# Trippasch/CudaRayTracer

Hardware: AMD Instinct MI355X
Metric: Mray/s (and ms/frame) at 1920x1080, 64 spp, depth 8, random-spheres (higher is better)
Workload: dtype f32; 1 GPU; c2: 1920x1080, 64 spp, depth 8, RTIOW final random-spheres scene; width=1920, height=1080, spp=64, depth=8, parallelism=1 GPU, kernel_variant=-1

## Files before the change

cudaraytracer_amd/_lib.py:

```python
from __future__ import annotations

import ctypes as C
import os

from . import abi

LIB_PATH = _IN_TREE = os.path.join(os.path.dirname(os.path.abspath(__file__)), "librt_hip.so")
LIB_PATH = os.environ.get("RT_HIP_LIB", LIB_PATH)

EXPORTED = [
    "LaunchKernel",
    "LaunchRandInit",
    "LaunchRenderInit",
    "rt_last_error",
    "rt_version",
    "rt_abi_version",
    "rt_set_launch_flags",
    "rt_set_device",
    "rt_scene_create",
    "rt_scene_from_reference_graph",
    "rt_scene_update_materials",
    "rt_scene_destroy",
    "rt_scene_get_info",
    "rt_render_init",
    "rt_render_init_soa",
    "rt_soa_plane_words",
    "rt_render",
    "rt_tiled_create",
    "rt_tiled_render",
    "rt_tiled_destroy",
    "rt_gl_register_texture",
    "rt_gl_copy_image",
    "rt_gl_unregister",
    "rt_copy_image_to_host",
    "rt_write_ppm",
    "rt_set_timing",
    "rt_set_wave_trace",
    "rt_set_tile_order",
    "rt_set_pixel_cost",
    "rt_set_ray_dump",
    "rt_trace_rays",
    "rt_query_rays",
    "rt_gbuffer",
    "rt_denoise",
    "rt_denoise_scratch_bytes",
    "rt_temporal",
    "rt_temporal_dynamic",
    "rt_temporal_moments",
    "rt_denoise_variance",
    "rt_denoise_variance_scratch_bytes",
    "rt_scene_motion",
    "rt_scene_edit",
    "rt_last_kernel_ms",
    "rt_last_variant",
    "rt_last_launch_host_ms",
    "rt_set_variant",
    "rt_set_tuning",
    "rt_glibc_srand",
    "rt_glibc_rand_next",
    "rt_builtin_scene",
    "rt_camera_inputs",
    "rt_procedural_texture",
    "rt_reference_graph_flatten",
    "rt_build_host_tables",
    "rt_tile_entries_host",
    "rt_set_bounce_entries",
    "rt_bounce_entries_host",
    "rt_bounce_entry_cells",
]

_lib = None


class RTError(RuntimeError):
    pass


def _declare(lib: C.CDLL) -> None:
    P = C.POINTER
    vp = C.c_void_p
    lib.rt_last_error.restype = C.c_char_p
    lib.rt_version.restype = C.c_char_p
    lib.rt_set_launch_flags.argtypes = [C.c_uint32]
    lib.rt_set_device.argtypes = [C.c_int]
    lib.rt_scene_create.argtypes = [P(abi.SceneDesc), P(vp)]
    lib.rt_scene_from_reference_graph.argtypes = [vp, P(vp)]
    lib.rt_scene_update_materials.argtypes = [vp, P(abi.MaterialDesc), C.c_uint32]
    lib.rt_scene_destroy.argtypes = [vp]
    lib.rt_scene_get_info.argtypes = [vp, P(abi.SceneInfo)]
    lib.rt_render_init.argtypes = [vp, C.c_uint32, C.c_uint32, P(abi.Tiling), C.c_uint64, vp]
    lib.rt_render_init_soa.argtypes = [vp, C.c_uint32, C.c_uint32, P(abi.Tiling), C.c_uint64, vp]
    lib.rt_soa_plane_words.argtypes = [C.c_uint32, C.c_uint32]
    lib.rt_soa_plane_words.restype = C.c_uint64
    lib.rt_render.argtypes = [vp, P(abi.RenderArgs), vp]
    lib.rt_set_timing.argtypes = [C.c_int]
    lib.rt_tiled_create.argtypes = [P(abi.TiledDesc), P(abi.SceneDesc), P(vp)]
    lib.rt_tiled_render.argtypes = [vp, P(abi.TiledFrame), P(abi.TiledTiming)]
    lib.rt_tiled_destroy.argtypes = [vp]
    lib.rt_gl_register_texture.argtypes = [C.c_uint32, C.c_uint32, P(vp)]
    lib.rt_gl_copy_image.argtypes = [vp, vp, C.c_uint32, C.c_uint32, vp]
    lib.rt_gl_unregister.argtypes = [vp]
    lib.rt_copy_image_to_host.argtypes = [vp, vp, C.c_uint32, C.c_uint32, C.c_int, vp]
    lib.rt_write_ppm.argtypes = [C.c_char_p, vp, C.c_uint32, C.c_uint32, C.c_int]
    lib.rt_set_wave_trace.argtypes = [C.c_void_p, C.c_uint64]
    lib.rt_set_tile_order.argtypes = [C.c_void_p]
    lib.rt_set_pixel_cost.argtypes = [C.c_void_p, C.c_uint64]
    lib.rt_set_ray_dump.argtypes = [C.c_void_p, C.c_uint32, C.c_void_p, C.c_uint32]
    lib.rt_trace_rays.argtypes = [C.c_void_p, C.c_void_p, C.c_uint32, C.c_void_p, C.c_void_p, C.c_int, C.c_void_p]
    if LIB_PATH == _IN_TREE or hasattr(lib, "rt_query_rays"):
        lib.rt_query_rays.argtypes = [vp, P(abi.QueryArgs), vp]
    lib.rt_gbuffer.argtypes = [vp, P(abi.GBufferArgs), vp]
    lib.rt_denoise.argtypes = [P(abi.DenoiseArgs), vp]
    lib.rt_denoise_scratch_bytes.argtypes = [C.c_uint32, C.c_uint32, C.c_uint32]
    lib.rt_denoise_scratch_bytes.restype = C.c_uint64
    lib.rt_temporal.argtypes = [P(abi.TemporalArgs), vp]
    lib.rt_temporal_dynamic.argtypes = [P(abi.TemporalArgs), vp, C.c_uint32, vp]
    lib.rt_temporal_moments.argtypes = [P(abi.TemporalArgs), vp, C.c_uint32, vp, vp, vp]
    lib.rt_denoise_variance.argtypes = [P(abi.DenoiseVarianceArgs), vp]
    lib.rt_denoise_variance_scratch_bytes.argtypes = [C.c_uint32, C.c_uint32, C.c_uint32]
    lib.rt_denoise_variance_scratch_bytes.restype = C.c_uint64
    lib.rt_scene_motion.argtypes = [P(abi.HittableDesc), P(abi.HittableDesc), C.c_uint32, P(C.c_float)]
    lib.rt_scene_edit.argtypes = [vp, P(abi.HittableDesc), C.c_uint32, P(vp)]
    lib.rt_last_kernel_ms.restype = C.c_float
    lib.rt_last_variant.restype = C.c_int
    lib.rt_last_launch_host_ms.restype = C.c_float
    lib.rt_set_variant.argtypes = [C.c_int]
    lib.rt_set_tuning.argtypes = [C.c_int, C.c_int]
    lib.rt_glibc_srand.argtypes = [P(abi.GlibcRand), C.c_uint32]
    lib.rt_glibc_rand_next.argtypes = [P(abi.GlibcRand)]
    lib.rt_glibc_rand_next.restype = C.c_int32
    lib.rt_builtin_scene.argtypes = [C.c_int, C.c_uint32, P(abi.HittableDesc), P(C.c_uint32),
                                     P(abi.MaterialDesc), P(C.c_uint32)]
    lib.rt_procedural_texture.argtypes = [C.c_int, C.c_int32, C.c_int32, C.c_void_p]
    F3P = P(C.c_float)
    lib.rt_camera_inputs.argtypes = [F3P, F3P, F3P, C.c_float, C.c_float, C.c_float, F3P, F3P, P(abi.InputStruct)]
    lib.rt_reference_graph_flatten.argtypes = [vp, P(abi.HittableDesc), P(C.c_uint32), P(abi.MaterialDesc),
                                               P(C.c_uint32), P(abi.ImageDesc), P(C.c_uint32)]
    lib.rt_build_host_tables.argtypes = [P(abi.SceneDesc), P(C.c_float), P(C.c_float), P(C.c_float),
                                         P(C.c_int32), P(abi.HostTablesInfo)]
    if LIB_PATH == _IN_TREE or hasattr(lib, "rt_tile_entries_host"):
        lib.rt_tile_entries_host.argtypes = [P(abi.SceneDesc), P(abi.InputStruct), C.c_uint32, C.c_uint32, P(abi.Tiling),
                                             C.c_uint32, C.c_uint32, C.c_uint32, P(C.c_uint32)]
    if LIB_PATH == _IN_TREE or hasattr(lib, "rt_set_bounce_entries"):
        lib.rt_set_bounce_entries.argtypes = [C.c_int]
        lib.rt_bounce_entries_host.argtypes = [P(abi.SceneDesc), P(C.c_float), P(C.c_float), P(C.c_uint32), P(C.c_uint32),
                                               P(C.c_uint16), P(abi.BounceEntriesInfo)]
        lib.rt_bounce_entry_cells.argtypes = [P(abi.BounceEntriesInfo), P(C.c_float), C.c_uint32, P(C.c_uint32)]
    lib.LaunchKernel.argtypes = [vp, C.c_uint, C.c_uint, C.c_uint, C.c_uint, vp, vp, abi.InputStruct]
    lib.LaunchKernel.restype = None
    lib.LaunchRandInit.argtypes = [vp]
    lib.LaunchRandInit.restype = None
    lib.LaunchRenderInit.argtypes = [abi.Dim3, abi.Dim3, C.c_uint, C.c_uint, vp]
    lib.LaunchRenderInit.restype = None


def lib() -> C.CDLL:
    global _lib
    if _lib is None:
        if not os.path.exists(LIB_PATH):
            raise RTError(f"{LIB_PATH} is missing: build it with `python -c 'import __graft_entry__ as g; g.build()'`")
        handle = C.CDLL(LIB_PATH)
        _declare(handle)
        _lib = handle
    return _lib


def check(rc: int, what: str) -> None:
    if rc != 0:
        msg = lib().rt_last_error().decode(errors="replace")
        raise RTError(f"{what} failed: {abi.STATUS.get(rc, rc)}: {msg}")
```

cudaraytracer_amd/csrc/render.hip:

```cpp
#include <hip/hip_runtime.h>

#include <cfloat>
#include <cstdio>
#include <cstdlib>
#include <cstring>
#include <atomic>
#include <map>
#include <numeric>
#include <memory>
#include <mutex>
#include <tuple>
#include <type_traits>
#include <vector>

#include "rt_epilogue.h"
#include "rt_internal.h"
#include "rt_scene_device.h"
#include "rt_tile_entry.h"

namespace rt {
namespace dev {

struct f3 {
    float x, y, z;
// ... 3381 lines not shown
    __syncthreads();
    for (uint32_t i = threadIdx.x; i < n; i += 1024u) order[atomicAdd(&start[cost_bucket(cost[i])], 1u)] = i;
}

__global__ __launch_bounds__(64) void tile_entries_kernel(const float* __restrict__ nodes, const float* __restrict__ prims,
                                                          const TileFrame F, TileRecord* __restrict__ out, const uint32_t n) {
    const uint32_t tile = blockIdx.x * 64u + threadIdx.x;
    if (tile < n) out[tile] = tile_record(nodes, prims, F, tile);
}

__global__ void rand_init_kernel(uint32_t* state) {
    if (threadIdx.x == 0 && blockIdx.x == 0) curand_init_state(1984ull, state);
}

}

namespace {

thread_local bool g_timing = false;
thread_local float g_last_ms = -1.0f;
thread_local float g_last_host_ms = -1.0f;
thread_local int g_variant = -1;
thread_local int g_last_variant = -1;

thread_local int g_regen_threshold = 56;
thread_local int g_regen_live_frac = 48;
thread_local int g_leaf_break = 3;
thread_local int g_lds_pad = 0;
thread_local int g_adaptive_order = 1;
thread_local int g_flat_max = 16;
thread_local int g_rius_trips = 4;
thread_local int g_rius_trips_persistent = 0;
thread_local int g_prefetch_stop = (int)dev::kPrefetchStop;
thread_local int g_persistent_waves = 0;
constexpr uint32_t kQueueMaxStride = 4096;
thread_local int g_queue_stride = 128;
thread_local int g_queue_chunk = 128;
thread_local int g_queue_prefetch = 32;
thread_local int g_queue_guide = 0;
thread_local int g_queue_min = 16;
thread_local int g_queue_host_reset = 0;
thread_local int g_persistent_group = 2;
thread_local int g_group_tail = 0;
thread_local int g_group_order = 0;
thread_local int g_group_chunk = 1024;
thread_local int g_group_waves = 16;
thread_local int g_group_linger_us = 0;
thread_local int g_tile_entries = 1;
thread_local int g_camera_resolve = 1;
constexpr uint32_t kCameraResolveCap = 8;
constexpr int kCameraResolveMax = 32;
thread_local int g_path_end_step = 1;
thread_local int g_bounce_entries = 1;

struct Knob {
    int& (*at)();
    int lo, hi, step;
    bool pow2;
    const char* refusal;
};
const Knob kKnobs[] = {
    {[]() -> int& { return g_regen_threshold; }, 1, 64, 1, false, "rt_set_tuning: regen threshold must be in [1, 64]"},
    {[]() -> int& { return g_leaf_max; }, 1, kLeafMax, 1, false, "rt_set_tuning: leaf max must be in [1, 4]"},
    {[]() -> int& { return g_persistent_waves; }, 0, 16, 1, false,
     "rt_set_tuning: persistent waves per SIMD must be in [0, 16]"},
    {[]() -> int& { return g_sah_traversal_x10; }, 1, 1000, 1, false,
     "rt_set_tuning: SAH traversal cost (x10) must be in [1, 1000]"},
    {[]() -> int& { return g_lds_pad; }, 0, 65536, 4, false, "rt_set_tuning: LDS pad must be a multiple of 4 in [0, 65536]"},
    {[]() -> int& { return g_adaptive_order; }, 0, 1, 1, false, "rt_set_tuning: adaptive order must be 0 or 1"},
    {[]() -> int& { return g_texel_bytes; }, 3, 4, 1, false, "rt_set_tuning: texel layout must be 3 (RGB8) or 4 (RGBA8)"},
    {[]() -> int& { return g_queue_chunk; }, 64, 4096, 64, false,
     "rt_set_tuning: queue chunk must be a multiple of 64 in [64, 4096]"},
    {[]() -> int& { return g_queue_stride; }, 128, (int)kQueueMaxStride, 1, true,
     "rt_set_tuning: queue head stride must be a power of two in [128, 4096] bytes"},
    {[]() -> int& { return g_regen_live_frac; }, 0, 64, 1, false, "rt_set_tuning: live fraction must be in [0, 64]"},
    {[]() -> int& { return g_leaf_break; }, 0, 64, 1, false, "rt_set_tuning: leaf break must be in [0, 64]"},
    {[]() -> int& { return g_rius_trips; }, 0, 64, 1, false, "rt_set_tuning: RandomInUnitSphere trips must be in [0, 64]"},
    {[]() -> int& { return g_flat_max; }, 0, (int)kFlatMaxPrims, 1, false,
     "rt_set_tuning: flat kernel primitive limit must be in [0, 64]"},
    {[]() -> int& { return g_queue_prefetch; }, 0, 64, 1, false, "rt_set_tuning: queue prefetch must be in [0, 64]"},
    {[]() -> int& { return g_queue_guide; }, 0, 64, 1, false, "rt_set_tuning: queue guide factor must be in [0, 64]"},
    {[]() -> int& { return g_queue_min; }, 16, 64, 16, false, "rt_set_tuning: guided chunk floor must be 16, 32, 48 or 64"},
    {[]() -> int& { return g_rius_trips_persistent; }, 0, 64, 1, false,
     "rt_set_tuning: RandomInUnitSphere trips must be in [0, 64]"},
    {[]() -> int& { return g_prefetch_stop; }, 0, 1024, 1, false, "rt_set_tuning: prefetch stop must be in [0, 1024]"},
    {[]() -> int& { return g_persistent_group; }, 0, 2, 1, false, "rt_set_tuning: persistent group must be 0, 1 or 2"},
    {[]() -> int& { return g_group_tail; }, 0, 1000, 1, false, "rt_set_tuning: group tail must be in [0, 1000] permille"},
    {[]() -> int& { return g_group_order; }, 0, 1, 1, false, "rt_set_tuning: group order must be 0 or 1"},
    {[]() -> int& { return g_queue_host_reset; }, 0, 1, 1, false, "rt_set_tuning: queue reset must be 0 or 1"},
    {[]() -> int& { return g_group_chunk; }, 64, 4096, 64, false,
     "rt_set_tuning: group chunk must be a multiple of 64 in [64, 4096]"},
    {[]() -> int& { return g_group_linger_us; }, 0, 100000, 1, false,
     "rt_set_tuning: group linger must be in [0, 100000] us"},
    {[]() -> int& { return g_group_waves; }, 4, 16, 4, false, "rt_set_tuning: group waves must be 4, 8, 12 or 16"},
    {[]() -> int& { return g_tile_entries; }, 0, 1, 1, false, "rt_set_tuning: tile entries must be 0 or 1"},
    {[]() -> int& { return g_camera_resolve; }, 0, kCameraResolveMax, 1, false,
     "rt_set_tuning: camera resolve must be 0, 1 or a primitive cap in [2, 32]"},
    {[]() -> int& { return g_path_end_step; }, 0, 1, 1, false, "rt_set_tuning: path end step must be 0 or 1"},
};
static_assert(sizeof(kKnobs) / sizeof(kKnobs[0]) == RT_TUNE_PATH_END_STEP + 1, "one row per rt_tuning_key");

int hip_check(hipError_t e, const char* what, int code = RT_ERR_DEVICE) {
    if (e == hipSuccess) return RT_OK;
    set_error(std::string(what) + ": " + hipGetErrorString(e));
    return code;
}
// ... 166 lines not shown
    TileFrame frame;
    ~EntryTable() {
        if (rec) (void)hipFree(rec);
    }
};
std::map<std::tuple<int, void*, uint32_t, uint32_t>, std::shared_ptr<EntryTable>>& g_entry_tables =
    *new std::map<std::tuple<int, void*, uint32_t, uint32_t>, std::shared_ptr<EntryTable>>();
std::mutex g_entry_tables_mu;

int acquire_entry_table(int device, hipStream_t s, uint32_t tiles_x, uint32_t tiles, std::shared_ptr<EntryTable>* out) {
    std::lock_guard<std::mutex> lock(g_entry_tables_mu);
    const auto key = std::make_tuple(device, (void*)s, tiles_x, tiles);
    auto it = g_entry_tables.find(key);
    if (it == g_entry_tables.end()) {
        if (g_entry_tables.size() >= kMaxPlans) g_entry_tables.clear();
        auto t = std::make_shared<EntryTable>();
        void* r = nullptr;
        const int rc = hip_check(hipMalloc(&r, (size_t)tiles * sizeof(TileRecord)), "rt_render: tile entry allocation");
        if (rc != RT_OK) return rc;
        t->rec = (TileRecord*)r;
        it = g_entry_tables.emplace(key, std::move(t)).first;
    }
    *out = it->second;
    return RT_OK;
}

TileFrame tile_frame_of(const dev::KParams& P, const bool wide_refs, const uint32_t depth) {
    TileFrame F;
    std::memset(&F, 0, sizeof(F));
    for (int i = 0; i < 3; i++) {
        F.origin[i] = P.origin[i];
        F.up[i] = P.up[i];
        F.right[i] = P.right[i];
        F.fov_fwd[i] = P.fov_fwd[i];
        F.k10_fwd[i] = P.k10_fwd[i];
    }
    F.near_plane = P.near_plane;
    F.far_plane = P.far_plane;
    F.width_f = P.width_f;
    F.cx = P.cx;
    F.cy = P.cy;
    F.width = P.width;
    F.local_rows = P.local_rows;
    F.band_rows = P.band_rows;
    F.num_ranks = P.num_ranks;
    F.rank = P.rank;
    F.grid_w = P.grid_w;
    F.grid_h = P.grid_h;
    F.tiles_x = P.tiles_x;
    F.num_nodes = P.num_nodes;
    F.num_prims = P.num_prims;
    F.wide_refs = wide_refs ? 1u : 0u;
    F.max_entries = std::min<uint32_t>(kTileEntryMax, depth + 2u);
    return F;
}

constexpr size_t kLdsLimit = 160 * 1024;
constexpr size_t kFlatTabLdsMax = 16 * 1024;

constexpr uint32_t kQueueSlots = 256;
constexpr int kMaxDevices = 64;
struct QueueRing {
    uint32_t* buf = nullptr;
    size_t slot_bytes = 0;
    std::atomic<uint32_t> next{0};
    int cus = 0;
    std::vector<void*> retired;
};
QueueRing g_queues[kMaxDevices];
std::mutex g_queue_mu;

int acquire_queue(int device, uint32_t stride, uint32_t** head, int* cus) {
    if (device < 0 || device >= kMaxDevices) {
        set_error("rt_render: device ordinal out of range");
        return RT_ERR_DEVICE;
    }
    QueueRing& q = g_queues[device];
    const size_t need = (size_t)dev::kQueueSlotWords * stride;
    std::lock_guard<std::mutex> lock(g_queue_mu);
    if (!q.buf || q.slot_bytes < need) {
        if (q.buf) {
            q.retired.push_back(q.buf);
            q.buf = nullptr;
        }
        void* p = nullptr;
        int rc = hip_check(hipMalloc(&p, (size_t)kQueueSlots * need), "rt_render: work queue allocation");
        if (rc != RT_OK) return rc;
        rc = hip_check(hipMemset(p, 0, (size_t)kQueueSlots * need), "rt_render: work queue reset");
        if (rc == RT_OK) rc = hip_check(hipDeviceSynchronize(), "rt_render: work queue reset");
        if (rc != RT_OK) {
            (void)hipFree(p);
            return rc;
        }
        q.buf = (uint32_t*)p;
        q.slot_bytes = need;
        if (q.cus == 0) {
            int n = 0;
            rc = hip_check(hipDeviceGetAttribute(&n, hipDeviceAttributeMultiprocessorCount, device),
                           "rt_render: compute unit count");
            if (rc != RT_OK) return rc;
            q.cus = n;
        }
    }
    *head = q.buf + (size_t)(q.next.fetch_add(1u) % kQueueSlots) * (q.slot_bytes / 4u);
    *cus = q.cus;
    return RT_OK;
// ... 145 lines not shown
        k10 = k10 * 10.0f;
        for (int i = 0; i < 3; i++) {
            P.origin[i] = in.origin[i];
            P.up[i] = in.up[i];
            P.fov_fwd[i] = in.fov * fw[i];
            P.k10_fwd[i] = k10 * fw[i];
            P.bg0[i] = in.background_start[i];
            P.bg1[i] = in.background_end[i];
        }
    }
}

int rt_tile_entries_host(const rt_scene_desc* desc, const rt_input_struct* inputs, uint32_t width, uint32_t height,
                         const rt_tiling* tiling, uint32_t flags, uint32_t first_tile, uint32_t num_tiles,
                         uint32_t* records) {
    if (!desc || !inputs || !tiling || (num_tiles && !records)) {
        set_error("rt_tile_entries_host: NULL argument");
        return RT_ERR_INVALID_ARGUMENT;
    }
    if (!tiling_ok(*tiling) || width == 0 || height == 0) {
        set_error("rt_tile_entries_host: invalid frame or tiling");
        return RT_ERR_INVALID_ARGUMENT;
    }
    HostScene h;
    try {
        std::string err;
        const int rc = build_host_scene(desc, &h, &err, false);
        if (rc != RT_OK) {
            set_error("rt_tile_entries_host: " + err);
            return rc;
        }
    } catch (const std::exception& e) {
        set_error(std::string("rt_tile_entries_host: ") + e.what());
        return RT_ERR_INVALID_ARGUMENT;
    }
    dev::KParams P;
    std::memset(&P, 0, sizeof(P));
    P.num_nodes = h.num_nodes;
    P.num_prims = h.num_prims;
    fill_frame(P, width, height, *tiling, (flags & RT_FLAG_FAITHFUL_GRID) != 0);
    P.tiles_x = (width + 7u) / 8u;
    fill_camera(P, *inputs, width, height);
    const uint64_t tiles = (uint64_t)P.tiles_x * ((tiling->local_rows + 7u) / 8u);
    if ((uint64_t)first_tile + num_tiles > tiles) {
        set_error("rt_tile_entries_host: tiles outside the frame");
        return RT_ERR_INVALID_ARGUMENT;
    }
    const TileFrame F = tile_frame_of(P, h.wide_refs, h.depth);
    for (uint32_t i = 0; i < num_tiles; i++) {
        const TileRecord r = tile_record(h.nodes.data(), h.prims.data(), F, first_tile + i);
        std::memcpy(records + 4 * (size_t)i, r.w, 16);
    }
    return RT_OK;
}

static uint32_t auto_rays_per_lane(const uint32_t n) {
    return (uint32_t)std::max<uint64_t>(1, std::min<uint64_t>(16, (uint64_t)n / (64ull * 8192ull)));
}

int rt_trace_rays(const rt_scene* scene, const float* rays, uint32_t n, int32_t* hits, uint64_t* counters,
                  int count_tests, rt_stream stream) {
    if (!scene || (n && (!rays || !hits))) { set_error("rt_trace_rays: NULL argument"); return RT_ERR_INVALID_ARGUMENT; }
    if (n == 0) return RT_OK;
    const DeviceScene& S = scene->dev;
    const size_t lds = (size_t)(S.depth + 2) * 64 * (S.wide_refs ? 4 : 2);
    if (S.depth > (uint32_t)dev::kStackMax || lds > kLdsLimit) { set_error("rt_trace_rays: BVH too deep"); return RT_ERR_UNSUPPORTED; }
    dev::KParams P;
    std::memset(&P, 0, sizeof(P));
    fill_scene_tables(P, S);
    P.counters = (unsigned long long*)counters;
    P.regen_threshold = (uint32_t)g_regen_threshold;
    P.regen_live_frac = (uint32_t)g_regen_live_frac;
    P.leaf_break = (uint32_t)g_leaf_break;
    const uint32_t per_wave = 64u * auto_rays_per_lane(n);
    const uint32_t grid = (uint32_t)(((uint64_t)n + per_wave - 1) / per_wave);
    hipStream_t s = (hipStream_t)stream;
    (void)hipGetLastError();
    const bool count = count_tests && counters;
    const auto kernel = S.wide_refs ? (count ? dev::trace_rays_kernel<true, true> : dev::trace_rays_kernel<false, true>)
                                    : (count ? dev::trace_rays_kernel<true, false> : dev::trace_rays_kernel<false, false>);
    hipLaunchKernelGGL(kernel, dim3(grid), dim3(64), lds, s, P, (const float4*)rays, n, per_wave, (int2*)hits);
    return hip_check(hipGetLastError(), "rt_trace_rays: kernel launch", RT_ERR_LAUNCH);
}

int rt_gbuffer(const rt_scene* scene, const rt_gbuffer_args* a, rt_stream stream) {
    if (!a) { set_error("rt_gbuffer: NULL args"); return RT_ERR_INVALID_ARGUMENT; }
    if (a->reserved[0] != 0 || a->reserved[1] != 0) { set_error("rt_gbuffer: reserved fields must be 0"); return RT_ERR_INVALID_ARGUMENT; }
    if (!a->normal_depth && !a->albedo && !a->prim_id) { set_error("rt_gbuffer: no output buffer"); return RT_ERR_INVALID_ARGUMENT; }
    if (!scene) { set_error("rt_gbuffer: NULL scene"); return RT_ERR_INVALID_ARGUMENT; }
    const rt_tiling& T = a->tiling;
    if (a->width == 0 || a->height == 0 || T.local_rows == 0) return RT_OK;
    int rc = check_tiling("rt_gbuffer", T);
    if (rc == RT_OK) rc = check_last_row("rt_gbuffer", T, a->height);
    if (rc != RT_OK) return rc;
    const DeviceScene& S = scene->dev;
    const bool flat = S.prims_flat && S.flat_source && S.num_prims <= (uint32_t)g_flat_max;
    const size_t lds = flat ? 0 : (size_t)(S.depth + 2) * 64 * (S.wide_refs ? 4 : 2);
    if (S.depth > (uint32_t)dev::kStackMax || lds > kLdsLimit) { set_error("rt_gbuffer: BVH too deep"); return RT_ERR_UNSUPPORTED; }
    dev::GBufParams G;
    std::memset(&G, 0, sizeof(G));
    dev::KParams& P = G.K;
    fill_scene_tables(P, S);
    if (flat) fill_flat_tables(P, S);
    fill_frame(P, a->width, a->height, T, false);
    P.leaf_break = (uint32_t)g_leaf_break;
    fill_camera(P, a->inputs, a->width, a->height);
// ... 55 lines not shown
    Q.material = a->material;
    Q.hits = (int2*)a->hits;
    Q.source = (const int32_t*)S.prim_source;
    Q.n = a->n;
    Q.per_wave = 64u * (a->rays_per_lane ? a->rays_per_lane : auto_rays_per_lane(a->n));
    const uint32_t grid = (uint32_t)((n + Q.per_wave - 1) / Q.per_wave);
    hipStream_t s = (hipStream_t)stream;
    (void)hipGetLastError();
    if (S.wide_refs)
        hipLaunchKernelGGL(dev::query_rays_kernel<true>, dim3(grid), dim3(64), lds, s, Q);
    else
        hipLaunchKernelGGL(dev::query_rays_kernel<false>, dim3(grid), dim3(64), lds, s, Q);
    return hip_check(hipGetLastError(), "rt_query_rays: kernel launch", RT_ERR_LAUNCH);
}

int rt_set_pixel_cost(void* buffer, uint64_t bytes) {
    g_pixel_cost = (bytes && buffer) ? (uint8_t*)buffer : nullptr;
    g_pixel_cost_bytes = g_pixel_cost ? bytes : 0;
    return RT_OK;
}

int rt_set_tile_order(const void* order) {
    g_tile_order = (const uint32_t*)order;
    return RT_OK;
}

int rt_set_timing(int enabled) {
    g_timing = enabled != 0;
    return RT_OK;
}

float rt_last_kernel_ms(void) { return g_last_ms; }

float rt_last_launch_host_ms(void) { return g_last_host_ms; }

int rt_set_variant(int variant) {
    int prev = g_variant;
    g_variant = variant;
    return prev;
}

int rt_last_variant(void) { return g_last_variant; }

int rt_set_bounce_entries(int on) {
    if (on != 0 && on != 1) {
        set_error("rt_set_bounce_entries: the value must be 0 or 1");
        return RT_ERR_INVALID_ARGUMENT;
    }
    const int prev = g_bounce_entries;
    g_bounce_entries = on;
    return prev;
}

int rt_set_tuning(int key, int value) {
    if (key < 0 || key >= (int)(sizeof(kKnobs) / sizeof(kKnobs[0]))) {
        set_error("rt_set_tuning: unknown key");
        return RT_ERR_INVALID_ARGUMENT;
    }
    const Knob& k = kKnobs[key];
    if (value < k.lo || value > k.hi || value % k.step || (k.pow2 && (value & (value - 1)))) {
        set_error(k.refusal);
        return RT_ERR_INVALID_ARGUMENT;
    }
    int& knob = k.at();
    const int prev = knob;
    knob = value;
    return prev;
}

namespace {

int check_render_args(const rt_scene& scene, const rt_render_args& a) {
    const auto refuse = [](const char* what) -> int {
        set_error(what);
        return RT_ERR_INVALID_ARGUMENT;
    };
    const bool philox = (a.flags & RT_FLAG_RNG_PHILOX) != 0;
    if (!a.state && !philox) return refuse("rt_render: state is NULL");
    if (philox && a.samples_per_pixel > RT_PHILOX_MAX_SPP)
        return refuse("rt_render: RT_FLAG_RNG_PHILOX supports at most RT_PHILOX_MAX_SPP (16384) samples per pixel");
    if (a.reserved != 0 || a.reserved2 != 0) return refuse("rt_render: reserved fields must be 0");
    if (!a.pos && !a.radiance && !a.accum) return refuse("rt_render: no output buffer");
    if ((a.flags & RT_FLAG_ACCUMULATE) && !a.accum) return refuse("rt_render: ACCUMULATE without accum");
    if ((a.flags & RT_FLAG_ACCUMULATE_RESET) && !(a.flags & RT_FLAG_ACCUMULATE))
        return refuse("rt_render: ACCUMULATE_RESET without ACCUMULATE");
    int rc = check_tiling("rt_render", a.tiling);
    if (rc == RT_OK) rc = check_last_row("rt_render", a.tiling, a.height);
    if (rc != RT_OK) return rc;
    if (scene.dev.depth > (uint32_t)dev::kStackMax) {
        set_error("rt_render: BVH deeper than the traversal stack");
        return RT_ERR_UNSUPPORTED;
    }
    return RT_OK;
}

int fill_render_params(dev::KParams& P, const DeviceScene& S, const rt_render_args& a) {
    std::memset(&P, 0, sizeof(P));
    fill_scene_tables(P, S);
    P.bvh_ref_nodes = (const float4*)S.bvh_ref_nodes;
    P.bvh_boxes = (const float4*)S.bvh_boxes;
    P.bvh_ref_pairs = (const float4*)S.bvh_ref_pairs;
    P.bvh_has_rects = S.has_rects ? 1u : 0u;
    P.pos = a.pos;
    P.radiance = (float4*)a.radiance;
    P.accum = (float4*)a.accum;
    P.state = (uint32_t*)a.state;
// ... 410 lines not shown
```

cudaraytracer_amd/csrc/rt_tile_entry.h:

```cpp
#pragma once

#include <cmath>
#include <cstdint>

#include "../../include/rt_hip.h"

#if defined(__HIPCC__)
#define RT_TILE_HD __host__ __device__
#else
#define RT_TILE_HD
#endif

namespace rt {

constexpr uint32_t kTileEntryMax = 8;
constexpr uint32_t kTileEntryRoot = 0u;
constexpr uint32_t kTileEntryNone = 0x7fffu;
constexpr uint32_t kTileEntryStack = 64;

struct TileRecord {
    uint32_t w[4];
};

struct TileFrame {
    float origin[3], up[3], right[3], fov_fwd[3], k10_fwd[3];
    float near_plane, far_plane, width_f, cx, cy;
    uint32_t width, local_rows, band_rows, num_ranks, rank;
    uint32_t grid_w, grid_h;
    uint32_t tiles_x;
    uint32_t num_nodes, num_prims;
    uint32_t wide_refs;
    uint32_t max_entries;
};

RT_TILE_HD inline TileRecord tile_record_root() {
    const uint32_t pad = kTileEntryNone | (kTileEntryNone << 16);
    return TileRecord{{kTileEntryRoot | (kTileEntryNone << 16), pad, pad, pad}};
}

RT_TILE_HD inline bool tile_finite(const float v) { return v - v == 0.0f; }

RT_TILE_HD inline TileRecord tile_record(const float* nodes, const float* prims, const TileFrame& F, const uint32_t tile) {
    const TileRecord root = tile_record_root();
    if (F.num_nodes == 0 || F.wide_refs || F.tiles_x == 0 || F.band_rows == 0 || F.band_rows % 8u != 0) return root;
    if (F.max_entries < 1 || F.max_entries > kTileEntryMax) return root;
    const uint32_t bx = tile % F.tiles_x, by = tile / F.tiles_x;
    const uint32_t x0 = bx * 8u, ly0 = by * 8u;
    if (x0 + 8u > F.width || x0 + 8u > F.grid_w || ly0 + 8u > F.local_rows) return root;
    const uint32_t band = ly0 / F.band_rows, within = ly0 - band * F.band_rows;
    const uint64_t g0l = ((uint64_t)band * F.num_ranks + F.rank) * F.band_rows + within;
    if (g0l + 8u > F.grid_h) return root;
    const float g0 = (float)(int)(uint32_t)g0l;
    const float near = F.near_plane, span = F.far_plane - F.near_plane;
    bool ok = tile_finite(near) && tile_finite(span) && span != 0.0f && tile_finite(F.width_f) && F.width_f > 0.0f &&
              tile_finite(F.cx) && tile_finite(F.cy);
    for (int a = 0; a < 3; a++)
        ok = ok && tile_finite(F.origin[a]) && tile_finite(F.up[a]) && tile_finite(F.right[a]) &&
             tile_finite(F.fov_fwd[a]) && tile_finite(F.k10_fwd[a]);
    if (!ok) return root;
    const float s_e = -near / span;
    if (!(s_e <= 0.0f) || !tile_finite(s_e)) return root;
    const float u_lo = ((float)(int)x0 - 1.0f - F.cx) / F.width_f, u_hi = ((float)(int)x0 + 9.0f - F.cx) / F.width_f;
    const float v_lo = (F.cy - (g0 + 8.0f)) / F.width_f, v_hi = (F.cy - g0 + 2.0f) / F.width_f;
    const float cu[4] = {u_lo, u_hi, u_hi, u_lo}, cv[4] = {v_lo, v_lo, v_hi, v_hi};
    float E[3], D[4][3], Dc[3], Dmax = 0.0f;
    for (int a = 0; a < 3; a++) {
        const float A = F.k10_fwd[a] - F.fov_fwd[a];
        E[a] = F.origin[a] + F.fov_fwd[a] + s_e * A;
        for (int k = 0; k < 4; k++) D[k][a] = A + span * (cu[k] * F.right[a] + cv[k] * F.up[a]);
        Dc[a] = 0.25f * ((D[0][a] + D[1][a]) + (D[2][a] + D[3][a]));
        ok = ok && tile_finite(E[a]);
    }
    float N[4][3];
    for (int k = 0; k < 4; k++) {
        const float* p = D[k];
        const float* q = D[(k + 1) & 3];
        float n[3] = {p[1] * q[2] - p[2] * q[1], p[2] * q[0] - p[0] * q[2], p[0] * q[1] - p[1] * q[0]};
        float len = 0.0f;
        for (int a = 0; a < 3; a++) len += n[a] * n[a];
        const float side = n[0] * Dc[0] + n[1] * Dc[1] + n[2] * Dc[2];
        if (!(len > 0.0f) || !tile_finite(len) || side == 0.0f) return root;
        const float inv = (side < 0.0f ? -1.0f : 1.0f) / sqrtf(len);
        for (int a = 0; a < 3; a++) N[k][a] = n[a] * inv;
        Dmax = fmaxf(Dmax, fmaxf(fabsf(p[0]), fmaxf(fabsf(p[1]), fabsf(p[2]))));
    }
    if (!ok || !tile_finite(Dmax)) return root;
    for (int k = 0; k < 4; k++)
        for (int j = 0; j < 4; j++) {
            const float d = N[k][0] * D[j][0] + N[k][1] * D[j][1] + N[k][2] * D[j][2];
            if (!(d >= -0x1p-16f * Dmax)) return root;
        }
    const auto meets = [&](const float lx, const float hx, const float ly, const float hy, const float lz,
                           const float hz) -> bool {
        for (int k = 0; k < 4; k++) {
            const float* n = N[k];
            const float px = n[0] >= 0.0f ? hx : lx, py = n[1] >= 0.0f ? hy : ly, pz = n[2] >= 0.0f ? hz : lz;
            const float d = n[0] * (px - E[0]) + n[1] * (py - E[1]) + n[2] * (pz - E[2]);
            const float mag = fabsf(n[0]) * (fabsf(px) + fabsf(E[0])) + fabsf(n[1]) * (fabsf(py) + fabsf(E[1])) +
                              fabsf(n[2]) * (fabsf(pz) + fabsf(E[2]));
            if (d < -0x1p-18f * mag) return false;
        }
        return true;
    };
    const auto prim_meets = [&](const float* p) -> bool {
        uint32_t tag;
        __builtin_memcpy(&tag, p + 7, 4);
        const uint32_t type = tag & 15u;
        if (type == RT_SPHERE) {
            const float rad = fabsf(p[3]) * (1.0f + 0x1p-16f);
            for (int k = 0; k < 4; k++) {
                const float* n = N[k];
                const float d = n[0] * (p[0] - E[0]) + n[1] * (p[1] - E[1]) + n[2] * (p[2] - E[2]);
                const float mag = fabsf(n[0]) * (fabsf(p[0]) + fabsf(E[0])) + fabsf(n[1]) * (fabsf(p[1]) + fabsf(E[1])) +
                                  fabsf(n[2]) * (fabsf(p[2]) + fabsf(E[2]));
                if (d < -(rad + 0x1p-18f * mag)) return false;
            }
            return true;
        }
        const float k0 = p[0] - 0.0001f - 0x1p-16f * fabsf(p[0]), k1 = p[0] + 0.0001f + 0x1p-16f * fabsf(p[0]);
        if (type == RT_XYRECT) return meets(p[1], p[2], p[3], p[4], k0, k1);
        if (type == RT_XZRECT) return meets(p[1], p[2], k0, k1, p[3], p[4]);
        if (type == RT_YZRECT) return meets(k0, k1, p[1], p[2], p[3], p[4]);
        return true;
    };
    uint32_t e[kTileEntryMax];
    for (uint32_t i = 0; i < kTileEntryMax; i++) e[i] = kTileEntryNone;
    uint32_t n_e = 0, sp = 0;
    int32_t stack[kTileEntryStack];
    int32_t node = 0;
    for (;;) {
        if ((uint32_t)node >= F.num_nodes) return root;
        const float* r = nodes + (size_t)node * 16;
        int32_t c[2];
        __builtin_memcpy(&c[0], r + 12, 4);
        __builtin_memcpy(&c[1], r + 13, 4);
        const bool m[2] = {meets(r[0], r[1], r[2], r[3], r[8], r[9]), meets(r[4], r[5], r[6], r[7], r[10], r[11])};
        int32_t next = -1;
        for (int k = 0; k < 2; k++) {
            if (!m[k]) continue;
            if (c[k] < 0) {
                const uint32_t l = ~(uint32_t)c[k], first = l >> 2, count = (l & 3u) + 1u;
                if (first + count > F.num_prims) return root;
                uint32_t run = 0;
                for (uint32_t j = 0; j <= count; j++) {
                    if (j < count && prim_meets(prims + (size_t)(first + j) * 8)) {
                        run++;
                        continue;
                    }
                    if (run) {
                        if (n_e == F.max_entries) return root;
                        e[n_e++] = ~(((first + j - run) << 2) | (run - 1u)) & 0xffffu;
                        run = 0;
                    }
                }
            } else if (next < 0) {
                next = c[k];
            } else {
                if (sp == kTileEntryStack) return root;
                stack[sp++] = c[k];
            }
        }
        if (next < 0) {
            if (sp == 0) break;
            next = stack[--sp];
        }
        node = next;
    }
    return TileRecord{{e[0] | (e[1] << 16), e[2] | (e[3] << 16), e[4] | (e[5] << 16), e[6] | (e[7] << 16)}};
}

}
```

cudaraytracer_amd/renderer.py:

```python
from __future__ import annotations

import ctypes as C

import numpy as np
import torch

from . import abi
from ._lib import RTError, check, lib
from .scenes import Scene


class DeviceScene:

    def __init__(self, scene: Scene | None = None, reference_graph: int | None = None):
        L = lib()
        self.handle = C.c_void_p()
        self.scene = scene
        if reference_graph is not None:
            check(L.rt_scene_from_reference_graph(C.c_void_p(reference_graph), C.byref(self.handle)),
                  "rt_scene_from_reference_graph")
        else:
            self._desc = scene.desc()
            check(L.rt_scene_create(C.byref(self._desc), C.byref(self.handle)), "rt_scene_create")

# ... 6 lines not shown
        check(lib().rt_scene_update_materials(self.handle, C.cast(materials, C.POINTER(abi.MaterialDesc)),
                                              len(materials)), "rt_scene_update_materials")

    def edited(self, hittables) -> "DeviceScene":
        from .scenes import _hittable_array
        new = DeviceScene.__new__(DeviceScene)
        new.handle = C.c_void_p()
        arr = _hittable_array(hittables)
        new.scene = None
        if self.scene is not None:
            copy = (abi.HittableDesc * len(arr)).from_buffer_copy(arr)
            new.scene = Scene(copy, self.scene.materials, self.scene.images)
        check(lib().rt_scene_edit(self.handle, arr, len(arr), C.byref(new.handle)), "rt_scene_edit")
        return new

    QUERY_OUTPUTS = {"normal_depth": ((4,), torch.float32), "albedo": ((4,), torch.float32), "prim_id": ((), torch.int32),
                     "uv": ((2,), torch.float32), "material": ((), torch.int32), "hits": ((2,), torch.int32)}

    def query(self, rays, outputs=("normal_depth", "albedo", "prim_id", "uv", "material", "hits"),
              rays_per_lane: int = 0) -> dict:
        names = tuple(outputs)
        unknown = [o for o in names if o not in self.QUERY_OUTPUTS]
        if unknown or not names or len(set(names)) != len(names):
            raise ValueError(f"outputs must be distinct names out of {tuple(self.QUERY_OUTPUTS)}, not {names!r}")
        if isinstance(rays, np.ndarray):
            rays = torch.from_numpy(np.array(rays, dtype=np.float32, order="C")).cuda()
        if rays.dtype != torch.float32 or rays.dim() != 3 or tuple(rays.shape[1:]) != (2, 4) or not rays.is_cuda:
            raise ValueError("rays must be a float32 (n, 2, 4) tensor on the device")
        rays = rays.contiguous()
        n = rays.shape[0]
        out = {o: torch.empty((n,) + self.QUERY_OUTPUTS[o][0], dtype=self.QUERY_OUTPUTS[o][1], device=rays.device)
               for o in names}
        if n == 0:
            return out
        a = abi.QueryArgs()
        a.rays = rays.data_ptr()
        for o in names:
            setattr(a, o, out[o].data_ptr())
        a.n, a.rays_per_lane = n, rays_per_lane
        stream = torch.cuda.current_stream(rays.device).cuda_stream
        check(lib().rt_query_rays(self.handle, C.byref(a), C.c_void_p(stream)), "rt_query_rays")
        return out

    def close(self) -> None:
        if self.handle:
            lib().rt_scene_destroy(self.handle)
            self.handle = C.c_void_p()

    def __del__(self):
        try:
            self.close()
        except Exception:
            pass


def band_rows_of(height: int, band_rows: int, num_ranks: int, rank: int) -> list[int]:
    rows = []
    b = rank
    while b * band_rows < height:
        rows.extend(range(b * band_rows, min(height, (b + 1) * band_rows)))
        b += num_ranks
    return rows


class Renderer:

    def __init__(self, width: int, height: int, device: int | str = 0, band_rows: int | None = None,
                 num_ranks: int = 1, rank: int = 0, rng: str = "xorwow", state_layout: str = "curand"):
        if rng not in ("xorwow", "philox"):
            raise ValueError(f"rng must be 'xorwow' or 'philox', not {rng!r}")
        if state_layout not in ("curand", "soa"):
            raise ValueError(f"state_layout must be 'curand' or 'soa', not {state_layout!r}")
        self.state_layout = state_layout
        self.rng = rng
        self.seed = 1984
        self.frame = 0
        if not torch.cuda.is_available():
            raise RTError("no HIP device visible: librt_hip.so renders on MI355X only")
        self.device = torch.device("cuda", device) if isinstance(device, int) else torch.device(device)
        torch.cuda.set_device(self.device)
        check(lib().rt_set_device(self.device.index or 0), "rt_set_device")
        self.width, self.height = width, height
        self.band_rows = band_rows or height
        self.num_ranks, self.rank = num_ranks, rank
        self.rows = band_rows_of(height, self.band_rows, num_ranks, rank)
        self.local_rows = len(self.rows)
        n = width * self.local_rows
        self.pos = torch.zeros(n, dtype=torch.int32, device=self.device)
        words = n * abi.STATE_WORDS if state_layout == "curand" else 6 * int(lib().rt_soa_plane_words(width, self.local_rows))
        self.state = torch.zeros(words, dtype=torch.int32, device=self.device) if rng == "xorwow" else None
        self.counters = torch.zeros(abi.COUNTERS_WORDS, dtype=torch.int64, device=self.device)
        self.radiance = None
        self.accum = None
        self._accum_restart = False
        self.normal_depth = self.albedo = self.prim_id = None
        self.denoised = None
        self._denoise_scratch = None
        self._denoise_pos = None
        self.prev_normal_depth = self.prev_prim_id = self.prev_inputs = None
        self._gbuffer_inputs = None
        self.history = None
        self._history_spare = None
        self.motion = None
        self._temporal_pos = None
        self._prim_motion = None
        self.moments = None
# ... 265 lines not shown
```

include/rt_hip.h:

```cpp
#ifndef RT_HIP_H
#define RT_HIP_H

#include <stddef.h>
#include <stdint.h>

#ifdef __cplusplus
extern "C" {
#endif

typedef enum rt_status {
    RT_OK = 0,
    RT_ERR_INVALID_ARGUMENT = -1,
    RT_ERR_INVALID_SCENE = -2,
    RT_ERR_OUT_OF_MEMORY = -3,
    RT_ERR_DEVICE = -4,
    RT_ERR_LAUNCH = -5,
    RT_ERR_UNSUPPORTED = -6
} rt_status;

typedef enum rt_hittable_type {
    RT_SPHERE = 0,
    RT_XYRECT = 1,
    RT_XZRECT = 2,
    RT_YZRECT = 3
// ... 318 lines not shown
    uint64_t seed;
} rt_tiled_desc;

typedef struct rt_tiled_frame {
    uint32_t* pos;
    uint32_t samples_per_pixel;
    uint32_t max_depth;
    uint32_t flags;
    uint32_t rng_frame;
    uint32_t rng_frame_set;
    uint32_t reserved;
    rt_input_struct inputs;
} rt_tiled_frame;

typedef struct rt_tiled_timing {
    float render_ms;
    float gather_ms;
    float total_ms;
    uint32_t reserved;
    uint64_t rays;
} rt_tiled_timing;

int rt_tiled_create(const rt_tiled_desc* desc, const rt_scene_desc* scene, rt_tiled** out);
int rt_tiled_render(rt_tiled* tiled, const rt_tiled_frame* frame, rt_tiled_timing* timing);
int rt_tiled_destroy(rt_tiled* tiled);

typedef struct rt_gl_target rt_gl_target;

int rt_gl_register_texture(uint32_t gl_texture, uint32_t gl_target, rt_gl_target** out);
int rt_gl_copy_image(rt_gl_target* target, const uint32_t* device_pos, uint32_t width, uint32_t height,
                     rt_stream stream);
int rt_gl_unregister(rt_gl_target* target);

int rt_copy_image_to_host(uint32_t* host, const uint32_t* device_pos, uint32_t width, uint32_t height, int flip_rows,
                          rt_stream stream);

int rt_write_ppm(const char* path, const uint32_t* rgba, uint32_t width, uint32_t height, int flip_rows);


int rt_reference_graph_flatten(const void* world, rt_hittable_desc* hittables, uint32_t* num_hittables,
                               rt_material_desc* materials, uint32_t* num_materials, rt_image_desc* images,
                               uint32_t* num_images);

typedef struct rt_host_tables_info {
    uint32_t num_nodes, num_prims, num_materials, depth;
} rt_host_tables_info;
int rt_build_host_tables(const rt_scene_desc* desc, float* nodes, float* prims, float* materials,
                         int32_t* prim_source, rt_host_tables_info* info);

int rt_tile_entries_host(const rt_scene_desc* desc, const rt_input_struct* inputs, uint32_t width, uint32_t height,
                         const rt_tiling* tiling, uint32_t flags, uint32_t first_tile, uint32_t num_tiles,
                         uint32_t* records);

int rt_set_bounce_entries(int on);

typedef struct rt_bounce_entries_info {
    uint32_t num_nodes, num_chain_nodes, num_records, depth;
    uint32_t grid_dim[3];
    float grid_origin[3];
    float grid_inv[3];
    float grid_off[3];
} rt_bounce_entries_info;
int rt_bounce_entries_host(const rt_scene_desc* desc, float* chain_nodes, float* nodes48, uint32_t* refs,
                           uint32_t* records, uint16_t* grid, rt_bounce_entries_info* info);
int rt_bounce_entry_cells(const rt_bounce_entries_info* info, const float* origins, uint32_t n, uint32_t* cells);

typedef struct rt_glibc_rand { int32_t r[34]; uint32_t idx; } rt_glibc_rand;
void rt_glibc_srand(rt_glibc_rand* g, uint32_t seed);
int32_t rt_glibc_rand_next(rt_glibc_rand* g);

int rt_builtin_scene(int which, uint32_t seed, rt_hittable_desc* hittables, uint32_t* num_hittables,
                     rt_material_desc* materials, uint32_t* num_materials);

int rt_procedural_texture(int kind, int32_t width, int32_t height, uint8_t* rgb);

void rt_camera_inputs(const float position[3], const float orientation[3], const float world_up[3],
                      float fov_degrees, float near_plane, float far_plane, const float bg_start[3],
                      const float bg_end[3], rt_input_struct* out);

#ifdef __cplusplus
}
#endif

#endif
```

Measured before the change: 33520 Mray/s.

## Cull occluded sphere primitives from per-tile camera entry lists

Adds a conservative occlusion test to per-tile entry construction. For each 8x8 tile's ray cone it finds the nearest sphere that surely blocks every ray, then drops candidate primitives whose lower-bound hit distance lies beyond it. Surviving runs are re-encoded into the packed entry record, closing gaps when the run count would exceed the slot budget. This is meant to cut primary-ray intersection work for camera rays. In exchange it adds double-precision math per tile and relies on conservative epsilons for correctness. Also exposes a device-side entry-building entry point and a toggle, enabled by default.

```diff
diff --git a/cudaraytracer_amd/_lib.py b/cudaraytracer_amd/_lib.py
--- a/cudaraytracer_amd/_lib.py
+++ b/cudaraytracer_amd/_lib.py
@@ -64,6 +64,8 @@
     "rt_reference_graph_flatten",
     "rt_build_host_tables",
     "rt_tile_entries_host",
+    "rt_set_tile_occlusion",
+    "rt_tile_entries_device",
     "rt_set_bounce_entries",
     "rt_bounce_entries_host",
     "rt_bounce_entry_cells",
@@ -141,6 +143,10 @@
     if LIB_PATH == _IN_TREE or hasattr(lib, "rt_tile_entries_host"):
         lib.rt_tile_entries_host.argtypes = [P(abi.SceneDesc), P(abi.InputStruct), C.c_uint32, C.c_uint32, P(abi.Tiling),
                                              C.c_uint32, C.c_uint32, C.c_uint32, P(C.c_uint32)]
+    if LIB_PATH == _IN_TREE or hasattr(lib, "rt_set_tile_occlusion"):
+        lib.rt_set_tile_occlusion.argtypes = [C.c_int]
+        lib.rt_tile_entries_device.argtypes = [vp, P(abi.InputStruct), C.c_uint32, C.c_uint32, P(abi.Tiling), C.c_uint32,
+                                               vp, vp]
     if LIB_PATH == _IN_TREE or hasattr(lib, "rt_set_bounce_entries"):
         lib.rt_set_bounce_entries.argtypes = [C.c_int]
         lib.rt_bounce_entries_host.argtypes = [P(abi.SceneDesc), P(C.c_float), P(C.c_float), P(C.c_uint32), P(C.c_uint32),
diff --git a/cudaraytracer_amd/csrc/render.hip b/cudaraytracer_amd/csrc/render.hip
--- a/cudaraytracer_amd/csrc/render.hip
+++ b/cudaraytracer_amd/csrc/render.hip
@@ -3457,6 +3457,7 @@
 constexpr int kCameraResolveMax = 32;
 thread_local int g_path_end_step = 1;
 thread_local int g_bounce_entries = 1;
+thread_local int g_tile_occlusion = 1;
 
 struct Knob {
     int& (*at)();
@@ -3729,6 +3730,7 @@
     F.num_prims = P.num_prims;
     F.wide_refs = wide_refs ? 1u : 0u;
     F.max_entries = std::min<uint32_t>(kTileEntryMax, depth + 2u);
+    F.occlusion = g_tile_occlusion && g_camera_resolve == 1 ? 1u : 0u;
     return F;
 }
 
@@ -3980,6 +3982,36 @@
         std::memcpy(records + 4 * (size_t)i, r.w, 16);
     }
     return RT_OK;
+}
+
+int rt_tile_entries_device(const rt_scene* scene, const rt_input_struct* inputs, uint32_t width, uint32_t height,
+                           const rt_tiling* tiling, uint32_t flags, void* records, rt_stream stream) {
+    if (!scene || !inputs || !tiling || !records) {
+        set_error("rt_tile_entries_device: NULL argument");
+        return RT_ERR_INVALID_ARGUMENT;
+    }
+    if (!tiling_ok(*tiling) || width == 0 || height == 0) {
+        set_error("rt_tile_entries_device: invalid frame or tiling");
+        return RT_ERR_INVALID_ARGUMENT;
+    }
+    const DeviceScene& S = scene->dev;
+    dev::KParams P;
+    std::memset(&P, 0, sizeof(P));
+    P.num_nodes = S.num_nodes;
+    P.num_prims = S.num_prims;
+    fill_frame(P, width, height, *tiling, (flags & RT_FLAG_FAITHFUL_GRID) != 0);
+    P.tiles_x = (width + 7u) / 8u;
+    fill_camera(P, *inputs, width, height);
+    const uint64_t tiles = (uint64_t)P.tiles_x * ((tiling->local_rows + 7u) / 8u);
+    if (tiles == 0 || tiles > 0x7fffffffull) {
+        set_error("rt_tile_entries_device: tile count out of range");
+        return RT_ERR_INVALID_ARGUMENT;
+    }
+    const TileFrame F = tile_frame_of(P, S.wide_refs, S.depth);
+    (void)hipGetLastError();
+    hipLaunchKernelGGL(dev::tile_entries_kernel, dim3(((uint32_t)tiles + 63u) / 64u), dim3(64), 0, (hipStream_t)stream,
+                       (const float*)S.nodes, (const float*)S.prims, F, (TileRecord*)records, (uint32_t)tiles);
+    return hip_check(hipGetLastError(), "rt_tile_entries_device: kernel launch", RT_ERR_LAUNCH);
 }
 
 static uint32_t auto_rays_per_lane(const uint32_t n) {
@@ -4141,6 +4173,16 @@
     return prev;
 }
 
+int rt_set_tile_occlusion(int on) {
+    if (on != 0 && on != 1) {
+        set_error("rt_set_tile_occlusion: the value must be 0 or 1");
+        return RT_ERR_INVALID_ARGUMENT;
+    }
+    const int prev = g_tile_occlusion;
+    g_tile_occlusion = on;
+    return prev;
+}
+
 int rt_set_tuning(int key, int value) {
     if (key < 0 || key >= (int)(sizeof(kKnobs) / sizeof(kKnobs[0]))) {
         set_error("rt_set_tuning: unknown key");
diff --git a/cudaraytracer_amd/csrc/rt_tile_entry.h b/cudaraytracer_amd/csrc/rt_tile_entry.h
--- a/cudaraytracer_amd/csrc/rt_tile_entry.h
+++ b/cudaraytracer_amd/csrc/rt_tile_entry.h
@@ -31,6 +31,7 @@
     uint32_t num_nodes, num_prims;
     uint32_t wide_refs;
     uint32_t max_entries;
+    uint32_t occlusion;
 };
 
 RT_TILE_HD inline TileRecord tile_record_root() {
@@ -39,6 +40,108 @@
 }
 
 RT_TILE_HD inline bool tile_finite(const float v) { return v - v == 0.0f; }
+
+RT_TILE_HD inline uint32_t tile_mask_runs(const uint32_t m) {
+    const uint32_t s = m & ~(m << 1);
+    return (s & 1u) + (s >> 1 & 1u) + (s >> 2 & 1u) + (s >> 3 & 1u);
+}
+RT_TILE_HD inline uint32_t tile_mask_close_gap(uint32_t m) {
+    uint32_t j = 0;
+    while (j < 4u && !(m >> j & 1u)) j++;
+    while (j < 4u && (m >> j & 1u)) j++;
+    while (j < 4u && !(m >> j & 1u)) m |= 1u << j++;
+    return m;
+}
+
+struct TileSphereView {
+    double d, cos_t, sin_t, r, r_s, r_g, mag;
+};
+RT_TILE_HD inline bool tile_sphere_view(const float* p, const double E[3], const double axis[3], const double e_mag,
+                                        const double s_far, TileSphereView& s) {
+    if (!tile_finite(p[0]) || !tile_finite(p[1]) || !tile_finite(p[2]) || !tile_finite(p[3])) return false;
+    const double v[3] = {(double)p[0] - E[0], (double)p[1] - E[1], (double)p[2] - E[2]};
+    s.r = p[3] < 0.0f ? -(double)p[3] : (double)p[3];
+    s.d = sqrt(v[0] * v[0] + v[1] * v[1] + v[2] * v[2]);
+    if (!(s.d > 0.0) || !(s.r > 0.0)) return false;
+    s.cos_t = (v[0] * axis[0] + v[1] * axis[1] + v[2] * axis[2]) / s.d;
+    const double s2 = 1.0 - s.cos_t * s.cos_t;
+    s.sin_t = s2 > 0.0 ? sqrt(s2) : 0.0;
+    const double c1 = (p[0] < 0.0f ? -(double)p[0] : (double)p[0]) + (p[1] < 0.0f ? -(double)p[1] : (double)p[1]) +
+                      (p[2] < 0.0f ? -(double)p[2] : (double)p[2]);
+    s.mag = e_mag + c1 + s.r + s_far;
+    const double eps = 0x1p-18 * (s.mag * s.mag) / s.r;
+    s.r_s = s.r - (0x1p-10 * s.r + eps);
+    s.r_g = s.r + (0x1p-16 * s.r + eps);
+    return s.r_g - s.r_g == 0.0;
+}
+
+RT_TILE_HD inline void tile_occlusion(const float* prims, const float* E, const float (*D)[3], const float* Dc,
+                                      const float s_e, const uint32_t* run_first, const uint32_t* run_count,
+                                      uint32_t* run_keep, const uint32_t n_e) {
+    if (n_e == 1 && run_count[0] == 1) return;
+    const double Ed[3] = {(double)E[0], (double)E[1], (double)E[2]};
+    double axis[3] = {(double)Dc[0], (double)Dc[1], (double)Dc[2]};
+    const double alen = sqrt(axis[0] * axis[0] + axis[1] * axis[1] + axis[2] * axis[2]);
+    if (!(alen > 0.0) || alen - alen != 0.0) return;
+    for (int a = 0; a < 3; a++) axis[a] /= alen;
+    double cos_rho = 1.0, dlen_max = 0.0;
+    for (int k = 0; k < 4; k++) {
+        const double x = D[k][0], y = D[k][1], z = D[k][2];
+        const double len = sqrt(x * x + y * y + z * z);
+        if (!(len > 0.0)) return;
+        const double c = (x * axis[0] + y * axis[1] + z * axis[2]) / len;
+        if (!(c <= 1.0)) return;
+        if (c < cos_rho) cos_rho = c;
+        if (len > dlen_max) dlen_max = len;
+    }
+    cos_rho = 1.0 - ((1.0 - cos_rho) * (1.0 + 0x1p-8) + 0x1p-44);
+    if (!(cos_rho > 0.5)) return;
+    const double sin_rho = sqrt(1.0 - cos_rho * cos_rho);
+    const double s_far = -(double)s_e * dlen_max;
+    const double e_mag = (Ed[0] < 0.0 ? -Ed[0] : Ed[0]) + (Ed[1] < 0.0 ? -Ed[1] : Ed[1]) + (Ed[2] < 0.0 ? -Ed[2] : Ed[2]);
+    if (!(s_far >= 0.0) || s_far - s_far != 0.0 || e_mag - e_mag != 0.0) return;
+    double lower[kTileEntryMax * 4], mags[kTileEntryMax * 4];
+    double t_min = 0.0, mag_min = 0.0;
+    uint32_t a_k = kTileEntryMax * 4, k = 0;
+    for (uint32_t i = 0; i < n_e; i++)
+        for (uint32_t j = 0; j < run_count[i]; j++, k++) {
+            lower[k] = -1.0;
+            mags[k] = 0.0;
+            const float* p = prims + (size_t)(run_first[i] + j) * 8;
+            uint32_t tag;
+            __builtin_memcpy(&tag, p + 7, 4);
+            TileSphereView s;
+            if ((tag & 15u) != RT_SPHERE || !tile_sphere_view(p, Ed, axis, e_mag, s_far, s)) continue;
+            const double rs = s.r_s, rg = s.r_g, dd = s.d * s.d, cc = s.cos_t * cos_rho, ss = s.sin_t * sin_rho;
+            if (s.d > rg) {
+                const double c = s.cos_t >= cos_rho ? 1.0 : cc + ss;
+                const double s2 = 1.0 - c * c;
+                const double q = rg * rg - dd * (s2 > 0.0 ? s2 : 0.0);
+                if (q >= 0.0) {
+                    lower[k] = s.d * c - sqrt(q);
+                    mags[k] = s.mag;
+                }
+            }
+            if (!(rs > 0.0) || !(s.cos_t > 0.0)) continue;
+            if (!(s.d - rg > s_far + 0.016 + 0x1p-10 * s.mag)) continue;
+            const double c = cc - ss;
+            if (!(c > 0.0)) continue;
+            const double q = rs * rs - dd * (1.0 - c * c);
+            if (!(q > 0.0)) continue;
+            const double T = s.d * c - sqrt(q);
+            if (T - T != 0.0) continue;
+            if (a_k == kTileEntryMax * 4 || T < t_min) {
+                t_min = T;
+                mag_min = s.mag;
+                a_k = k;
+            }
+        }
+    if (a_k == kTileEntryMax * 4) return;
+    k = 0;
+    for (uint32_t i = 0; i < n_e; i++)
+        for (uint32_t j = 0; j < run_count[i]; j++, k++)
+            if (k != a_k && lower[k] > t_min * (1.0 + 0x1p-10) + 0x1p-18 * (mag_min + mags[k])) run_keep[i] &= ~(1u << j);
+}
 
 RT_TILE_HD inline TileRecord tile_record(const float* nodes, const float* prims, const TileFrame& F, const uint32_t tile) {
     const TileRecord root = tile_record_root();
@@ -123,8 +226,7 @@
         if (type == RT_YZRECT) return meets(k0, k1, p[1], p[2], p[3], p[4]);
         return true;
     };
-    uint32_t e[kTileEntryMax];
-    for (uint32_t i = 0; i < kTileEntryMax; i++) e[i] = kTileEntryNone;
+    uint32_t run_first[kTileEntryMax], run_count[kTileEntryMax], run_keep[kTileEntryMax];
     uint32_t n_e = 0, sp = 0;
     int32_t stack[kTileEntryStack];
     int32_t node = 0;
@@ -149,7 +251,9 @@
                     }
                     if (run) {
                         if (n_e == F.max_entries) return root;
-                        e[n_e++] = ~(((first + j - run) << 2) | (run - 1u)) & 0xffffu;
+                        run_first[n_e] = first + j - run;
+                        run_count[n_e] = run;
+                        run_keep[n_e++] = (1u << run) - 1u;
                         run = 0;
                     }
                 }
@@ -166,6 +270,31 @@
         }
         node = next;
     }
+    if (F.occlusion && n_e) tile_occlusion(prims, E, D, Dc, s_e, run_first, run_count, run_keep, n_e);
+    uint32_t refs = 0;
+    for (uint32_t i = 0; i < n_e; i++) refs += tile_mask_runs(run_keep[i]);
+    for (uint32_t i = 0; i < n_e && refs > n_e; i++)
+        while (refs > n_e && tile_mask_runs(run_keep[i]) > 1u) {
+            run_keep[i] = tile_mask_close_gap(run_keep[i]);
+            refs--;
+        }
+    uint32_t e[kTileEntryMax];
+    for (uint32_t i = 0; i < kTileEntryMax; i++) e[i] = kTileEntryNone;
+    uint32_t n_out = 0;
+    for (uint32_t i = 0; i < n_e; i++) {
+        uint32_t run = 0;
+        for (uint32_t j = 0; j <= run_count[i]; j++) {
+            if (j < run_count[i] && (run_keep[i] >> j & 1u)) {
+                run++;
+                continue;
+            }
+            if (run) {
+                if (n_out == kTileEntryMax) return root;
+                e[n_out++] = ~(((run_first[i] + j - run) << 2) | (run - 1u)) & 0xffffu;
+                run = 0;
+            }
+        }
+    }
     return TileRecord{{e[0] | (e[1] << 16), e[2] | (e[3] << 16), e[4] | (e[5] << 16), e[6] | (e[7] << 16)}};
 }
 
diff --git a/cudaraytracer_amd/renderer.py b/cudaraytracer_amd/renderer.py
--- a/cudaraytracer_amd/renderer.py
+++ b/cudaraytracer_amd/renderer.py
@@ -82,6 +82,13 @@
             self.close()
         except Exception:
             pass
+
+
+def set_tile_occlusion(on: bool) -> bool:
+    prev = lib().rt_set_tile_occlusion(1 if on else 0)
+    if prev < 0:
+        check(prev, "rt_set_tile_occlusion")
+    return bool(prev)
 
 
 def band_rows_of(height: int, band_rows: int, num_ranks: int, rank: int) -> list[int]:
diff --git a/include/rt_hip.h b/include/rt_hip.h
--- a/include/rt_hip.h
+++ b/include/rt_hip.h
@@ -394,6 +394,11 @@
                          const rt_tiling* tiling, uint32_t flags, uint32_t first_tile, uint32_t num_tiles,
                          uint32_t* records);
 
+int rt_set_tile_occlusion(int on);
+
+int rt_tile_entries_device(const rt_scene* scene, const rt_input_struct* inputs, uint32_t width, uint32_t height,
+                           const rt_tiling* tiling, uint32_t flags, void* records, rt_stream stream);
+
 int rt_set_bounce_entries(int on);
 
 typedef struct rt_bounce_entries_info {
```

Result: faster. 34780 Mray/s (median of 6 runs) (+3.8%).
